# bartelvdh/Navtex

Measured on AMD Instinct MI355X. Metric: IQ Msamples/s through FIR->FSK->bitsync, higher is better.
Workload: dtype f64

## Files before the change

### navtex_amd/__init__.py

```python
from __future__ import annotations

import ctypes as C
import os
from typing import Callable, Iterable, List, Optional, Sequence, Tuple

import numpy as np

from . import _native as N
from ._native import (CHAIN_490, CHAIN_518, FRAME_BITS, FRAME_IN, FRAME_RAW, FRAME_Y3, RATE_IN, RATE_RAW,
                      SOFT_DECODE, SOFT_KEEP, NvxError, lib)

__all__ = ["Pipeline", "Group", "Capture", "Sitor", "sitor_encode", "make_stream", "synth_host", "synth_device", "device_count",
           "DeviceBuffer", "channelise", "channelise_time_stats", "Store", "wav_write", "wav_read", "NvxError", "lib",
           "CHAIN_518", "CHAIN_490", "SOFT_DECODE", "SOFT_KEEP", "FRAME_BITS", "FRAME_IN", "FRAME_RAW", "FRAME_Y3", "RATE_IN", "RATE_RAW"]


def device_count() -> int:
    return lib.nvx_device_count()


def sitor_encode(text: str, n_phasing: int = 40) -> str:
    t = text.encode("ascii")
    n = lib.nvx_sitor_encode(t, n_phasing, None, 0)
    buf = C.create_string_buffer(n + 1)
# ... 210 lines not shown
        N.check(lib.nvx_get_carrier(self._h, stream, chain, C.byref(off), C.byref(ref)), "nvx_get_carrier")
        return off.value, bool(ref.value)

    def afc_enable(self, stream: int, chain: int, cfg: Optional[N.AfcConfig] = None, **fields) -> None:
        _afc_enable(lib.nvx_afc_enable, self._h, stream, chain, cfg, fields, "nvx_afc_enable")

    def afc_disable(self, stream: int, chain: int, keep: bool = False) -> None:
        N.check(lib.nvx_afc_disable(self._h, stream, chain, int(keep)), "nvx_afc_disable")

    def afc_status(self, stream: int, chain: int) -> dict:
        return _afc_status(lib.nvx_afc_read, self._h, stream, chain, "nvx_afc_read")

    def afc_trace(self, stream: int, chain: int) -> List[int]:
        return _afc_trace(lib.nvx_afc_trace, self._h, stream, chain, "nvx_afc_trace")

    def set_forms(self, independent: int = -1, dynamic_preroll: int = -1, demod_tiles: int = -1) -> None:
        N.check(lib.nvx_debug_set_forms(self._h, independent, dynamic_preroll, demod_tiles), "nvx_debug_set_forms")

    def last_forms(self) -> Tuple[int, int, int]:
        a, b, c = C.c_int(), C.c_int(), C.c_int()
        N.check(lib.nvx_debug_last_forms(self._h, C.byref(a), C.byref(b), C.byref(c)), "nvx_debug_last_forms")
        return a.value, b.value, c.value

    def _apply_forms(self, forms: Optional[Sequence[int]]) -> None:
        if forms is None:
            if not hasattr(lib, "nvx_debug_set_forms"):
                return
            forms = tuple(int(os.environ.get(name, -1)) for name in ("NVX_INDEPENDENT", "NVX_DYNAMIC_PREROLL", "NVX_DEMOD_TILES"))
        if tuple(forms) != (-1, -1, -1):
            self.set_forms(*forms)


class Pipeline(HandleStats):

    def __init__(self, n_streams: int = 1, raw_rate: bool = False, chain_mask: int = CHAIN_518 | CHAIN_490,
                 chain_masks: Optional[Iterable[int]] = None, labels: Optional[Sequence[Sequence[int]]] = None,
                 max_frames: int = 1, char_layer: bool = True, push_mode: bool = False, device: int = 0,
                 wideband: bool = False, bit_history: int = 0, store: "Optional[Store]" = None, stage0_order: int = 1,
                 eager_launch: bool = False, stall_timeout_ms: int = 0, forms: Optional[Sequence[int]] = None):
        self.messages: List[Tuple[int, int, str, str]] = []
        cfg = N.Config()
        lib.nvx_config_default(C.byref(cfg))
        cfg.device, cfg.n_streams, cfg.raw_rate = device, n_streams, int(raw_rate)
        cfg.stage0_order = int(stage0_order)
        cfg.eager_launch = int(eager_launch)
        cfg.stall_timeout_ms = int(stall_timeout_ms)
        cfg.chain_mask, cfg.max_frames, cfg.char_layer, cfg.push_mode = chain_mask, max_frames, int(char_layer), int(push_mode)
# ... 362 lines not shown
```

### navtex_amd/_native.py

```python
from __future__ import annotations

import ctypes as C
import os
from pathlib import Path

import numpy as np

_LIB_PATH = Path(os.environ.get("NAVTEX_AMD_LIB") or (Path(__file__).resolve().parent / "libnavtex_amd.so"))

OK, ERR_ARG, ERR_NODEV, ERR_HIP, ERR_NOMEM, ERR_STATE, ERR_IO = 0, -1, -2, -3, -4, -5, -6
RATE_RAW, RATE_IN = 2016000, 252000
FRAME_BITS, FRAME_IN, FRAME_RAW, FRAME_Y3 = 32, 80640, 645120, 288
CHAIN_518, CHAIN_490 = 1, 2
SOFT_DECODE, SOFT_KEEP = 1, 2
TUNE_N, TUNE_STEP_HZ, TUNE_MAX_HZ, TUNE_NOMINAL_K = 20160, 3.125, 25000.0, 4480

MESSAGE_FN = C.CFUNCTYPE(None, C.c_void_p, C.c_int, C.c_char_p, C.c_char_p, C.c_int)
SITOR_MSG_FN = C.CFUNCTYPE(None, C.c_void_p, C.c_char_p, C.c_char_p, C.c_int)
SITOR_TRACE_FN = C.CFUNCTYPE(None, C.c_void_p, C.c_char_p)


class Config(C.Structure):
    _fields_ = [
        ("struct_size", C.c_uint32), ("device", C.c_int), ("n_streams", C.c_int), ("raw_rate", C.c_int), ("chain_mask", C.c_uint32),
# ... 30 lines not shown
                ("min_samples", C.c_int), ("contrast_min", C.c_double)]


class AfcStatus(C.Structure):
    _fields_ = [("enabled", C.c_int), ("centre_k", C.c_int), ("k_last", C.c_int), ("last_step", C.c_int), ("offset_hz", C.c_double),
                ("launches", C.c_uint64), ("updates", C.c_uint64), ("held", C.c_uint64), ("clamped", C.c_uint64)]


AFC_TRACE_KEEP = 1024


def _load() -> C.CDLL:
    if not _LIB_PATH.exists():
        raise ImportError(
            f"{_LIB_PATH} is missing: build it with `python navtex_amd/build.py` "
            "(hipcc, gfx950). navtex_amd has no pure-Python or CPU fallback.")
    lib = C.CDLL(str(_LIB_PATH))
    vp, sz, i, u32 = C.c_void_p, C.c_size_t, C.c_int, C.c_uint32
    sig = {
        "nvx_last_error": (C.c_char_p, []), "nvx_version": (C.c_char_p, []), "nvx_abi_version": (i, []),
        "nvx_sample_to_int16": (i, [C.c_double, C.POINTER(C.c_int16)]), "nvx_shim_stats": (i, [C.POINTER(C.c_uint64), C.POINTER(C.c_uint64)]),
        "nvx_debug_advance_clock": (i, [vp, i, C.c_uint64]),
        "nvx_debug_set_forms": (i, [vp, i, i, i]), "nvx_debug_last_forms": (i, [vp, C.POINTER(i), C.POINTER(i), C.POINTER(i)]),
        "init_fir_filter1": (None, []), "sample_in_1": (None, [C.c_double, C.c_double]), "init_fir2_wrapper": (None, []),
        "nvx_set_trace": (i, [vp, SITOR_TRACE_FN, vp]),
        "nvx_shim_latency": (i, [C.POINTER(C.c_uint64), C.POINTER(C.c_double), C.POINTER(C.c_double), C.POINTER(C.c_double), C.POINTER(C.c_double), i]),
        "nvx_shim_flush": (i, []), "nvx_shim_finish": (i, []), "nvx_shim_bits": (sz, [i, C.c_char_p, sz]),
        "nvx_StreamACallback": (None, [vp, vp, vp, C.c_uint, C.c_uint, vp]),
        "nvx_capture_start": (i, [vp, i, C.c_double, C.POINTER(vp)]), "nvx_capture_callback": (None, [vp, vp, vp, C.c_uint, C.c_uint, vp]),
        "nvx_capture_latency": (i, [vp, C.POINTER(C.c_uint64), C.POINTER(C.c_double), C.POINTER(C.c_double), C.POINTER(C.c_double), C.POINTER(C.c_double), i]),
        "nvx_capture_stop": (i, [vp]), "nvx_capture_record": (i, [vp, C.c_char_p]), "nvx_fsm_selftest": (i, [u32, i]),
        "nvx_cascade_wait_stats": (i, [vp, C.POINTER(C.c_uint64), C.POINTER(C.c_uint64), C.POINTER(C.c_uint64), i]),
        "nvx_debug_cascade_state": (i, [vp, i, vp, sz, i]),
        "nvx_cascade_integrity_stats": (i, [vp, C.POINTER(C.c_uint64), C.POINTER(C.c_uint64), C.POINTER(C.c_uint64), i]), "nvx_capture_pause": (None, [vp, i]),
        "nvx_capture_stats": (None, [vp, C.POINTER(C.c_uint64), C.POINTER(C.c_uint64), C.POINTER(C.c_uint64)]),
        "nvx_config_default": (None, [C.POINTER(Config)]),
        "nvx_create": (i, [C.POINTER(Config), C.POINTER(vp)]), "nvx_destroy": (None, [vp]), "nvx_reset": (i, [vp]), "nvx_stream_reset": (i, [vp, i]),
        "nvx_push_iq": (i, [vp, i, vp, sz]), "nvx_push_planar": (i, [vp, i, vp, vp, sz]), "nvx_flush": (i, [vp]),
        "nvx_finish": (i, [vp]), "nvx_stream_finish": (i, [vp, i]),
        "nvx_poll_bits": (sz, [vp, i, i, C.c_char_p, sz]),
        "nvx_process_resident": (i, [vp, vp, sz, sz, i, vp]), "nvx_fetch_bits": (i, [vp]),
        "nvx_bit_count": (sz, [vp, i, i]),
        "nvx_last_kernel_ms": (C.c_float, [vp, i]), "nvx_enable_timing": (None, [vp, i]), "nvx_enable_debug": (i, [vp, i]),
        "nvx_group_create": (i, [C.POINTER(C.c_int), i, C.POINTER(Config), C.POINTER(vp)]), "nvx_group_destroy": (None, [vp]),
        "nvx_group_reset": (i, [vp]), "nvx_group_size": (i, [vp]),
        "nvx_group_member": (i, [vp, i, C.POINTER(i), C.POINTER(i), C.POINTER(i), C.POINTER(vp)]), "nvx_group_member_of": (i, [vp, i]),
# ... 81 lines not shown
```

### navtex_amd/csrc/nvx_api.cpp

```cpp
#include "nvx_handle.h"
#include <chrono>
#include <cmath>
#include "navtex_amd_afc.h"
#include "navtex_amd_signal.h"
#include "navtex_amd_soft.h"
#include "navtex_amd_tune.h"
#include "nvx_fsm.h"

extern "C" hipError_t nvx_launch_afc_update(const nvx_afc_args *a, hipStream_t s) __attribute__((weak));
static_assert(NVX_AFC_LAW_C == NVX_AFC_C && NVX_AFC_K_MAX * NVX_TUNE_STEP_HZ == NVX_TUNE_MAX_HZ, "the law's constants are the header's");
static_assert(sizeof(nvx_afc_note) == 8 && sizeof(nvx_afc_par) == 32, "layouts of nvx_afc_law.h");

static thread_local char g_err[512] = "";
extern "C" void nvx_set_error(const char *fmt, ...)
{
    va_list ap; va_start(ap, fmt);
    vsnprintf(g_err, sizeof g_err, fmt, ap);
    va_end(ap);
}
extern "C" const char *nvx_last_error(void) { return g_err; }
int64_t nvx_now_ns()
{
    return std::chrono::duration_cast<std::chrono::nanoseconds>(std::chrono::steady_clock::now().time_since_epoch()).count();
}
#define NVX_STR2(x) #x
#define NVX_STR(x) NVX_STR2(x)
// ... 127 lines not shown
        (void)hipFree(r.d_soft); r.d_soft = nullptr;
        (void)hipHostFree(r.h_soft); r.h_soft = nullptr;
        r.soft = false;
    }
    for (auto &s : h->slots) {
        if (s.soft_sitor) { nvx_sitor_free(s.soft_sitor); s.soft_sitor = nullptr; }
        s.soft_outbox.clear();
        std::vector<float>().swap(s.soft);
        s.soft_base = s.soft_polled = 0; s.soft_count = 0;
    }
    for (auto it = h->sinks.begin(); it != h->sinks.end();)
        if ((*it)->soft) { delete *it; it = h->sinks.erase(it); } else ++it;
    h->soft_mode = 0; h->soft_cap = 0;
}

static void free_handle(nvx_handle *h)
{
    if (!h) return;
    const std::string err = g_err;
    (void)hipSetDevice(h->cfg.device);
    (void)drain(h);
    snprintf(g_err, sizeof g_err, "%s", err.c_str());
    free_debug(h);
    free_afc(h);
    free_signal(h);
    free_soft(h);
    for (auto it = h->made.rbegin(); it != h->made.rend(); ++it) {
        switch (it->first) {
        case HipRes::stream: (void)hipStreamDestroy((hipStream_t)it->second); break;
        case HipRes::event:  (void)hipEventDestroy((hipEvent_t)it->second); break;
        case HipRes::device: (void)hipFree(it->second); break;
        case HipRes::pinned: (void)hipHostFree(it->second); break;
        }
    }
    for (auto &s : h->slots)
        if (s.sitor) nvx_sitor_free(s.sitor);
    for (auto *c : h->sinks) delete c;
    delete h;
}

extern "C" void nvx_destroy(nvx_handle *h) { free_handle(h); }

extern "C" int nvx_create(const nvx_config *cfg, nvx_handle **out)
{
    if (!cfg || !out) { nvx_set_error("nvx_create: null argument"); return NVX_ERR_ARG; }
    *out = nullptr;
// ... 290 lines not shown
        ca.n_frames = n_frames; ca.n_streams = n_here; ca.chain_masks = h->d_masks;
        ca.part = d_list;
        ca.state[0] = h->d_cstate[p0]; ca.state[1] = h->d_cstate[p0 ^ 1]; ca.y3 = h->d_y3[yb]; ca.y3_cap = (size_t)h->y3_cap; ca.y3_base = 0;
        ca.queue = h->d_ctrl; ca.status = h->d_ctrl + 1; ca.done = h->d_ctrl + NVX_CASCADE_CTRL_INTS;
        ca.stage0_order = h->cfg.stage0_order;
        ca.third0 = third0;
        ca.tune_k = afc ? h->d_afc_k[h->launched & 1] : h->d_tune_k;
        ca.max_waves_per_cu = -1;
        HIP_TRY(nvx_launch_cascade(&ca, h->cascade_raw, h->nch, &forms, st));
    }
    if (r.timed) HIP_TRY(hipEventRecord(r.ev[1], st));
    HIP_TRY(hipMemcpyAsync(h->h_status + NVX_STATUS_INTS * (h->launched % RESULT_SLOTS), h->d_ctrl + 1, NVX_STATUS_INTS * sizeof(int), hipMemcpyDeviceToHost, st));
    HIP_TRY(hipEventRecord(h->casc_done[yb], st));
    HIP_TRY(hipStreamWaitEvent(sd, h->casc_done[yb], 0));
    if (fused) {
        nvx_fir3_args fa{};
        fa.y2[0] = y2_bufs[0]; fa.y2[1] = y2_bufs[1]; fa.y2_pitch = h->y2_pitch; fa.y2_row = h->d_y2row;
        fa.y3 = h->d_y3[yb]; fa.y3_cap = (size_t)h->y3_cap; fa.y3_base = 0; fa.n_frames = n_frames; fa.n_slots = h->n_slots;
        fa.part = d_list; fa.n_part = r.n_part; fa.per_part = h->per_in;
        if (r.timed) HIP_TRY(hipEventRecord(r.ev[6], sd));
        HIP_TRY(nvx_launch_fir3(&fa, sd));
        if (r.timed) HIP_TRY(hipEventRecord(r.ev[7], sd));
    }
    if (r.timed) HIP_TRY(hipEventRecord(r.ev[2], sd));
    HIP_TRY(nvx_launch_demod_front(&da, sd));
    if (r.timed) HIP_TRY(hipEventRecord(r.ev[3], sd));
    if (!da.soft && !afc) HIP_TRY(hipEventRecord(h->demod_done[yb], sd));
    h->demod_pending[yb] = true;
    if (r.timed) HIP_TRY(hipEventRecord(r.ev[4], sd));
    HIP_TRY(nvx_launch_demod_fsm(&da, sd));
    if (r.timed) HIP_TRY(hipEventRecord(r.ev[5], sd));
    if (afc) {
        nvx_afc_args aa{};
        aa.sig = r.d_sig; aa.par = h->d_afc_par; aa.k_rw = h->d_afc_k[h->launched & 1]; aa.k_next = h->d_afc_k[(h->launched + 1) & 1];
        aa.note = r.d_note; aa.n_slots = h->n_slots; aa.part = d_list; aa.n_part = r.n_part;
        if (r.timed) HIP_TRY(hipEventRecord(r.ev[8], sd));
        HIP_TRY(nvx_launch_afc_update(&aa, sd));
        if (r.timed) HIP_TRY(hipEventRecord(r.ev[9], sd));
    }
    if (da.soft || afc) HIP_TRY(hipEventRecord(h->demod_done[yb], sd));
    HIP_TRY(hipMemcpyAsync(h->h_ties, h->d_ties, sizeof(nvx_tie_stats), hipMemcpyDeviceToHost, sd));
    HIP_TRY(hipMemcpyAsync(r.h_nbits, r.d_nbits, (size_t)h->n_slots * sizeof(int), hipMemcpyDeviceToHost, sd));
    HIP_TRY(hipMemcpyAsync(r.h_bits, r.d_bits, (size_t)h->n_slots * h->bits_cap, hipMemcpyDeviceToHost, sd));
    if (h->sig_on) HIP_TRY(hipMemcpyAsync(r.h_sig, r.d_sig, (size_t)h->n_slots * sizeof(nvx_sig_rec), hipMemcpyDeviceToHost, sd));
    r.sig = h->sig_on;
    if (afc) HIP_TRY(hipMemcpyAsync(r.h_note, r.d_note, (size_t)h->n_slots * sizeof(nvx_afc_note), hipMemcpyDeviceToHost, sd));
// ... 674 lines not shown
    if (periods > (~0ull - g_old) / (unsigned long long)NVX_CLOCK_PERIOD) { nvx_set_error("nvx_debug_advance_clock: the clock would pass 2^64"); return NVX_ERR_ARG; }
    const unsigned long long g_new = g_old + periods * (unsigned long long)NVX_CLOCK_PERIOD;
    const unsigned third_old = (unsigned)(g_old / (NVX_FRAME_Y3 / 3)), third_new = (unsigned)(g_new / (NVX_FRAME_Y3 / 3));
    unsigned long long seal[2];
    uint8_t *entry = h->d_cstate[h->parity[stream]] + (size_t)stream * NVX_CASCADE_STATE_BYTES + (size_t)NVX_STATE_SEAL * 16;
    HIP_TRY(hipMemcpy(seal, entry, sizeof seal, hipMemcpyDeviceToHost));
    seal[0] ^= seal_tag_host(stream, third_old) ^ seal_tag_host(stream, third_new);
    seal[1] = ((unsigned long long)(unsigned)stream << 32) | third_new;
    HIP_TRY(hipMemcpy(entry, seal, sizeof seal, hipMemcpyHostToDevice));
    h->g0s[stream] = g_new;
    h->diverged = !streams_together(h);
    return NVX_OK;
}

extern "C" int nvx_debug_set_forms(nvx_handle *h, int independent, int dynamic_preroll, int demod_tiles)
{
    const auto bad = [](int v) { return v < -1 || v > 1; };
    if (!h || bad(independent) || bad(dynamic_preroll) || bad(demod_tiles)) { nvx_set_error("nvx_debug_set_forms: null handle, or a value outside -1 (automatic), 0, 1"); return NVX_ERR_ARG; }
    std::lock_guard<std::mutex> lk(h->mu);
    h->forms_req = nvx_forms{ independent, dynamic_preroll, demod_tiles };
    return NVX_OK;
}

extern "C" int nvx_debug_last_forms(nvx_handle *h, int *independent, int *dynamic_preroll, int *front_tile_wgs)
{
    if (!h) { nvx_set_error("nvx_debug_last_forms: null handle"); return NVX_ERR_ARG; }
    std::lock_guard<std::mutex> lk(h->mu);
    if (!h->forms_known) { nvx_set_error("nvx_debug_last_forms: the handle has launched nothing yet"); return NVX_ERR_STATE; }
    if (independent) *independent = h->forms_last.independent;
    if (dynamic_preroll) *dynamic_preroll = h->forms_last.dynamic_preroll;
    if (front_tile_wgs) *front_tile_wgs = h->forms_last.demod_tiles;
    return NVX_OK;
}

extern "C" size_t nvx_debug_y3(nvx_handle *h, int stream, int chain, double *out, size_t cap_pairs)
{
    if (!h || !out || stream < 0 || stream >= h->n_streams || chain < 0 || chain > 1) return 0;
    std::lock_guard<std::mutex> lk(h->mu);
    hipSetDevice(h->cfg.device);
    hipDeviceSynchronize();
    size_t n = std::min(cap_pairs, (size_t)h->last_n3);
    const int in = stream / h->per_in;
    if (h->ended[in]) n = std::min(n, (size_t)(h->g0s[in] % NVX_FRAME_Y3));
    if (hipMemcpy(out, h->d_y3[(h->launched + 1) & 1] + (size_t)(2 * stream + chain) * h->y3_cap, n * sizeof(double2), hipMemcpyDeviceToHost) != hipSuccess) return 0;
    return n;
}
// ... 67 lines not shown
```

### navtex_amd/csrc/nvx_cascade.hip

```cpp
#include <hip/hip_runtime.h>
#include <stdint.h>
#include <stdlib.h>
#include <mutex>

#include "nvx_cascade_wave.h"
#include "nvx_tune_table.h"

__device__ double2 nvx_tune_tab[NVX_TUNE_TAB_ENTRIES];

__device__ __forceinline__ int add_low_halves(unsigned a, unsigned b)
{
    int r;
    asm("v_add_u32_sdwa %0, sext(%1), sext(%2) dst_sel:DWORD dst_unused:UNUSED_PAD src0_sel:WORD_0 src1_sel:WORD_0"
        : "=v"(r) : "v"(a), "v"(b));
    return r;
}
__device__ __forceinline__ int add_high_halves(unsigned a, unsigned b)
{
    int r;
    asm("v_add_u32_sdwa %0, sext(%1), sext(%2) dst_sel:DWORD dst_unused:UNUSED_PAD src0_sel:WORD_1 src1_sel:WORD_1"
        : "=v"(r) : "v"(a), "v"(b));
    return r;
}
__device__ __forceinline__ double stage0_component(u32x4 v, bool odd)
{
    const int sI = add_low_halves(v.x, v.y) + add_low_halves(v.z, v.w);
    const int sQ = add_high_halves(v.x, v.y) + add_high_halves(v.z, v.w);
    int mine = (odd ? sQ : sI) + 4;
// ... 240 lines not shown
template <bool RAW, int NCH>
__global__ __launch_bounds__(64) void nvx_fir_cascade(nvx_cascade_args a)
{
    if (RAW) cascade_wave_main<RAW, NCH, 1, const nvx_cascade_args &>(a);
    else cascade_wave_main<RAW, NCH, 1, const nvx_cascade_args>(a);
}

__global__ __launch_bounds__(64) __attribute__((amdgpu_waves_per_eu(3, 3))) void nvx_fir_cascade_cic3_1(nvx_cascade_args a) { cascade_wave_main<true, 1, 3, const nvx_cascade_args &>(a); }
__global__ __launch_bounds__(64) void nvx_fir_cascade_cic3_2(nvx_cascade_args a) { cascade_wave_main<true, 2, 3, const nvx_cascade_args &>(a); }

template <bool RAW, int NCH, int S0>
__global__ __launch_bounds__(64) void nvx_fir_cascade_list(nvx_cascade_args a)
{
    if (RAW) cascade_wave_main<RAW, NCH, S0, const nvx_cascade_args &, true>(a);
    else cascade_wave_main<RAW, NCH, S0, const nvx_cascade_args, true>(a);
}

template <bool RAW, int NCH, int S0, bool LIST> struct CascadeKernel { static constexpr auto fn = nvx_fir_cascade_list<RAW, NCH, S0>; };
template <bool RAW, int NCH> struct CascadeKernel<RAW, NCH, 1, false> { static constexpr auto fn = nvx_fir_cascade<RAW, NCH>; };
template <> struct CascadeKernel<true, 1, 3, false> { static constexpr auto fn = nvx_fir_cascade_cic3_1; };
template <> struct CascadeKernel<true, 2, 3, false> { static constexpr auto fn = nvx_fir_cascade_cic3_2; };

#define NVX_MAX_DEVICES 64
template <bool RAW, int NCH, int S0 = 1, bool LIST = false>
static hipError_t launch_cascade_as(const nvx_cascade_args *a, nvx_forms *f, hipStream_t s)
{
    static std::mutex mu;
    static int cus_of[NVX_MAX_DEVICES], fit_of[NVX_MAX_DEVICES];
    int n_cus = 0, fit_per_cu = 0;
    {
        int dev = 0;
        hipError_t e = hipGetDevice(&dev);
        if (e != hipSuccess) return e;
        std::lock_guard<std::mutex> lk(mu);
        const bool cached = dev >= 0 && dev < NVX_MAX_DEVICES && cus_of[dev] > 0;
        if (!cached) {
            int cus = 0, per_cu = 0;
            e = hipDeviceGetAttribute(&cus, hipDeviceAttributeMultiprocessorCount, dev);
            if (e == hipSuccess) e = hipOccupancyMaxActiveBlocksPerMultiprocessor(&per_cu, CascadeKernel<RAW, NCH, S0, LIST>::fn, 64, 0);
            if (e != hipSuccess) return e;
            n_cus = cus; fit_per_cu = per_cu > 0 ? per_cu : 1;
            if (dev >= 0 && dev < NVX_MAX_DEVICES) { cus_of[dev] = n_cus; fit_of[dev] = fit_per_cu; }
        } else {
            n_cus = cus_of[dev]; fit_per_cu = fit_of[dev];
        }
    }
    int per_cu = fit_per_cu;
    if (a->max_waves_per_cu > 0 && a->max_waves_per_cu < per_cu) per_cu = a->max_waves_per_cu;
    if (a->max_waves_per_cu < 0 && per_cu + a->max_waves_per_cu >= 4) per_cu += a->max_waves_per_cu;
    const int resident = n_cus * per_cu;
    nvx_cascade_args args = *a;
    args.independent = f->independent >= 0 ? f->independent : (a->n_streams < resident && a->n_frames > 1);
    const long long whole_units = (long long)a->n_streams * a->n_frames;
    const int split_frames = whole_units > resident ? 1 : ((args.independent && 3 * whole_units <= resident) ? a->n_frames : 0);
    args.split_from = a->n_frames - split_frames;
    const long long units = (long long)a->n_streams * (args.split_from + 3LL * split_frames);
    const unsigned grid = (unsigned)(units < resident ? units : resident);
    args.dynamic_preroll = f->dynamic_preroll != 0;
    f->independent = args.independent; f->dynamic_preroll = args.dynamic_preroll;
    hipLaunchKernelGGL((CascadeKernel<RAW, NCH, S0, LIST>::fn), dim3(grid), dim3(64), 0, s, args);
    return hipGetLastError();
}

static hipError_t tune_table_ready()
{
    static std::mutex mu;
    static bool done[NVX_MAX_DEVICES];
    int dev = 0;
    hipError_t e = hipGetDevice(&dev);
    if (e != hipSuccess) return e;
    if (dev < 0 || dev >= NVX_MAX_DEVICES) return hipErrorInvalidDevice;
    std::lock_guard<std::mutex> lk(mu);
    if (done[dev]) return hipSuccess;
    double2 *tab = (double2 *)calloc(NVX_TUNE_TAB_ENTRIES, sizeof(double2));
    if (!tab) return hipErrorOutOfMemory;
    for (int j = 0; j < NVX_TUNE_TAB_N; j++) nvx_tune_entry(j, &tab[j].x, &tab[j].y);
    for (int o = 0; o < NVX_MIX_N; o++) {
        const int j = (NVX_TUNE_NOMINAL_K * o) % NVX_TUNE_TAB_N;
        tab[NVX_TUNE_TAB_N + j] = double2{ NVX_MIX_CR[o], NVX_MIX_CI[o] };
        tab[2 * NVX_TUNE_TAB_N + (NVX_TUNE_TAB_N - j) % NVX_TUNE_TAB_N] = double2{ NVX_MIX_CR[o], -NVX_MIX_CI[o] };
    }
    e = hipMemcpyToSymbol(HIP_SYMBOL(nvx_tune_tab), tab, NVX_TUNE_TAB_ENTRIES * sizeof(double2), 0, hipMemcpyHostToDevice);
    free(tab);
// ... 20 lines not shown
```

### navtex_amd/csrc/nvx_demod.hip

```cpp
#include <hip/hip_runtime.h>
#include <stdint.h>
#include <stdlib.h>

#include "nvx_tables.h"
#include "nvx_atan2.h"
#include "nvx_fsm.h"
#include "nvx_kernels.h"

enum { DS_Y3 = 0, DS_DPHI = 8, DS_S = 16, DS_C = 24, DS_COUNT = 24 + 567 };
enum { DI_SYNCED = 0, DI_SYNC_OFF, DI_NEXT_SYNC_OFF, DI_PHASE, DI_PREV_OFFSET, DI_COUNT };
static_assert(DI_COUNT == NVX_DEMOD_INTS && DS_COUNT == NVX_DEMOD_DOUBLES && DI_PREV_OFFSET == NVX_DI_PREV_OFFSET &&
              DI_PHASE == NVX_DI_PHASE, "state layout");

#ifndef NVX_FRONT_THREADS
#define NVX_FRONT_THREADS 128
#endif
#ifndef DTL
#define DTL NVX_FRONT_TILE
static_assert(DTL % 9 == 0, "a tile is a whole number of bit periods");
#endif
#define FRONT_SLIDE ((567 + NVX_FRONT_THREADS - 1) / NVX_FRONT_THREADS)
#define G_DAB 8
#define G_CB 574
#define G_CSA 582

__device__ __forceinline__ double2 y3_at(const double2 *y3, const double *hist, int t)
{
    if (t >= 0) return y3[t];
    double2 r; r.x = hist[2 * (4 + t)]; r.y = hist[2 * (4 + t) + 1];
    return r;
// ... 129 lines not shown
    c.slot = chain_index; c.g0 = a.g0; c.n3 = a.n3;
    int parity = 0;
    if (a.part) {
        const int per = 2 * a.per_part, e = chain_index / per;
        c.slot = a.part[e].stream * per + (chain_index - e * per);
        c.g0 = a.part[e].g0; parity = a.part[e].parity; c.n3 = a.part[e].n3;
    }
    c.st_rd = (parity ? a.dstate[1] : a.dstate[0]) + (size_t)c.slot * NVX_DEMOD_DOUBLES;
    c.st_wr = (parity ? a.dstate[0] : a.dstate[1]) + (size_t)c.slot * NVX_DEMOD_DOUBLES;
    return c;
}

__device__ __forceinline__ void front_publish_ties(const nvx_demod_args &a, const FrontTies &t, unsigned *s_near, unsigned *s_evals, unsigned *s_minm, int tid)
{
    if (t.evals) { atomicAdd(s_near, t.near); atomicAdd(s_evals, t.evals); atomicMin(s_minm, __float_as_uint(t.minm)); }
    __syncthreads();
    if (tid == 0 && *s_evals) {
        if (*s_near) atomicAdd(&a.ties->near_ties, (unsigned long long)*s_near);
        atomicAdd(&a.ties->evaluations, (unsigned long long)*s_evals);
        atomicMin(&a.ties->min_margin_bits, *s_minm);
    }
}

struct FrontWalkLds {
    double dphi[8 + DTL];
    double S[8 + DTL];
    double C[567 + DTL];
    unsigned char D[DTL];
    unsigned near, evals, minm;
    FrontSig sig[NVX_FRONT_THREADS / 64];
};
template <bool SIG>
__device__ __forceinline__ void front_sequential(const nvx_demod_args &a, int chain_index, int n_tiles_here, FrontWalkLds &lds)
{
    double *const s_dphi = lds.dphi, *const s_S = lds.S, *const s_C = lds.C;
    unsigned char *const s_D = lds.D;
    unsigned &s_near = lds.near, &s_evals = lds.evals, &s_minm = lds.minm;
    const int tid = threadIdx.x;
    const FrontChain ch = front_chain(a, chain_index);
    const int slot = ch.slot;
    if (!a.slot_active[slot]) return;
    if (tid == 0) { s_near = 0; s_evals = 0; s_minm = 0x7f800000u; }
    FrontTies ties = front_ties_init();
    constexpr bool sig_on = SIG;
    FrontSig sig;
    front_sig_init(sig);

    const double *st = ch.st_rd;
    const double2 *y3 = a.y3 + (size_t)slot * a.y3_cap + a.y3_base;
    double *dphi_out = a.dphi ? a.dphi + (size_t)slot * a.y3_cap + a.y3_base : nullptr;
    double *corr_out = a.corr ? a.corr + (size_t)slot * a.y3_cap + a.y3_base : nullptr;
    double *csum_out = a.csum ? a.csum + (size_t)slot * a.y3_cap + a.y3_base : nullptr;
    const double *hist = st + DS_Y3;
    if (tid < 8) { s_dphi[tid] = st[DS_DPHI + tid]; s_S[tid] = st[DS_S + tid]; }
    for (int i = tid; i < 567; i += NVX_FRONT_THREADS) s_C[i] = st[DS_C + i];
    __syncthreads();

    const int n3 = ch.n3;
    const int n_here = n_tiles_here > 0 ? min(n3, n_tiles_here * DTL) : n3;
    for (int ta = 0; ta < n_here; ta += DTL) {
        const int tl = min(DTL, n_here - ta);
        const int tl9 = (tl + 8) / 9;
        const unsigned long long gt = ch.g0 + (unsigned long long)ta;
        for (int L = tid; L < tl; L += NVX_FRONT_THREADS) {
            const int t = ta + L;
            const double2 w3 = y3_at(y3, hist, t - 1), w4 = y3[t];
            const double ds = front_dphi(w4, w3);
            s_dphi[8 + L] = ds;
            if (dphi_out) dphi_out[t] = ds;
            float hi, lo;
            const unsigned char d = front_decision(y3_at(y3, hist, t - 4), y3_at(y3, hist, t - 3), y3_at(y3, hist, t - 2), w3, w4, hi, lo);
            s_D[L] = d;
            if (sig_on && gt + L >= G_DAB) front_sig_add(sig, w4, ds, d, hi, lo);
        }
        if (tid < 9 * tl9 - tl) s_D[tl + tid] = 0;
        __syncthreads();
        for (int L = tid; L < tl; L += NVX_FRONT_THREADS)
            s_C[567 + L] = (gt + L >= G_DAB) ? front_corr(&s_dphi[L]) : 0.0;
        __syncthreads();
        const unsigned t_cb = (unsigned)((gt % 5103u + (5103u - G_CB % 5103u)) % 5103u);
        for (int L = tid; L < tl; L += NVX_FRONT_THREADS)
            s_S[8 + L] = (gt + L >= G_CB) ? front_class_sum(&s_C[567 + L], t_cb + (unsigned)L) : 0.0;
        __syncthreads();
        if (corr_out)
            for (int L = tid; L < tl; L += NVX_FRONT_THREADS) { corr_out[ta + L] = s_C[567 + L]; csum_out[ta + L] = s_S[8 + L]; }
        for (int M = tid; M < tl9; M += NVX_FRONT_THREADS) {
            const int L = 9 * M + (G_CSA % 9);
// ... 3 lines not shown
        double h_d = 0.0, h_s = 0.0, h_c[FRONT_SLIDE];
        if (tid < 8) { h_d = s_dphi[tl + tid]; h_s = s_S[tl + tid]; }
#pragma unroll
        for (int k = 0; k < FRONT_SLIDE; k++) { const int i = tid + NVX_FRONT_THREADS * k; h_c[k] = (i < 567) ? s_C[tl + i] : 0.0; }
        __syncthreads();
        if (tid < 8) { s_dphi[tid] = h_d; s_S[tid] = h_s; }
#pragma unroll
        for (int k = 0; k < FRONT_SLIDE; k++) { const int i = tid + NVX_FRONT_THREADS * k; if (i < 567) s_C[i] = h_c[k]; }
        __syncthreads();
    }

    front_publish_ties(a, ties, &s_near, &s_evals, &s_minm, tid);
    if (sig_on) {
        const unsigned skip = ch.g0 >= G_DAB ? 0u : (unsigned)min((unsigned long long)n_here, G_DAB - ch.g0);
        front_sig_publish(sig, (unsigned)n_here - skip, lds.sig, a.sig_part + (size_t)slot * a.sig_stride, tid);
    }
    if (n_tiles_here > 0) return;
    double *sw = ch.st_wr;
    if (tid < 4 && n3 >= 4) { const double2 l = y3[n3 - 4 + tid]; sw[DS_Y3 + 2 * tid] = l.x; sw[DS_Y3 + 2 * tid + 1] = l.y; }
    if (tid < 8) { sw[DS_DPHI + tid] = s_dphi[tid]; sw[DS_S + tid] = s_S[tid]; }
    for (int i = tid; i < 567; i += NVX_FRONT_THREADS) sw[DS_C + i] = s_C[i];
}

__global__ __launch_bounds__(NVX_FRONT_THREADS) __attribute__((amdgpu_waves_per_eu(5))) void nvx_demod_front(nvx_demod_args a)
{
    __shared__ FrontWalkLds lds;
    if (a.sig) front_sequential<true>(a, blockIdx.x, 0, lds);
    else front_sequential<false>(a, blockIdx.x, 0, lds);
}

#define FRONT_LOOKBACK 576
__global__ __launch_bounds__(NVX_FRONT_THREADS) void nvx_demod_front_head(nvx_demod_args a)
{
    __shared__ FrontWalkLds lds;
    if (a.sig) front_sequential<true>(a, blockIdx.x, 2, lds);
    else front_sequential<false>(a, blockIdx.x, 2, lds);
}
__global__ __launch_bounds__(NVX_FRONT_THREADS) void nvx_demod_front_tiles(nvx_demod_args a, int wgs_per_chain)
{
    const int chain_index = blockIdx.x / wgs_per_chain, wg = blockIdx.x - chain_index * wgs_per_chain;
    __shared__ double p_dphi[FRONT_LOOKBACK + DTL];
    __shared__ double p_C[FRONT_LOOKBACK - 8 + DTL];
    __shared__ double p_S[2 + DTL];
    __shared__ unsigned char p_D[DTL];
    __shared__ unsigned s_near, s_evals, s_minm;
    __shared__ FrontSig s_sig[NVX_FRONT_THREADS / 64];
    const int tid = threadIdx.x;
    const FrontChain ch = front_chain(a, chain_index);
    const int slot = ch.slot;
    if (!a.slot_active[slot]) return;
    if (tid == 0) { s_near = 0; s_evals = 0; s_minm = 0x7f800000u; }
// ... 208 lines not shown
    {
        const uint4 *src = (const uint4 *)a.fsm_table;
        uint4 *dst = (uint4 *)s_tab;
        for (int i = threadIdx.x; i < NVX_FSM_TABLE_ALLOC / 4; i += 64) dst[i] = src[i];
    }
    __syncthreads();
    if (a.soft) fsm_chain<true>(a, s_tab);
    else fsm_chain<false>(a, s_tab);
}

extern "C" int nvx_front_tile_wgs(const nvx_demod_args *a, int request)
{
    const unsigned chains = a->part ? (unsigned)(2 * a->per_part * a->n_part) : (unsigned)a->n_slots;
    const int tiles = (a->n3 + DTL - 1) / DTL;
    const long long chain_frames = (long long)chains * (a->n3 / NVX_Y3_PER_FRAME);
    const bool parallel = tiles >= 3 && (request >= 0 ? request != 0 : chain_frames <= 2560);
    return parallel ? tiles - 2 : 0;
}

extern "C" hipError_t nvx_launch_demod_front(const nvx_demod_args *a, hipStream_t s)
{
    const unsigned chains = a->part ? (unsigned)(2 * a->per_part * a->n_part) : (unsigned)a->n_slots;
    const int wgs = a->sig_parts - 1;
    if (wgs < 0) return hipErrorInvalidValue;
    if (a->sig && 1 + wgs > a->sig_stride) return hipErrorInvalidValue;
    if (wgs) {
        hipLaunchKernelGGL(nvx_demod_front_head, dim3(chains), dim3(NVX_FRONT_THREADS), 0, s, *a);
        hipLaunchKernelGGL(nvx_demod_front_tiles, dim3(chains * (unsigned)wgs), dim3(NVX_FRONT_THREADS), 0, s, *a, wgs);
    } else {
        hipLaunchKernelGGL(nvx_demod_front, dim3(chains), dim3(NVX_FRONT_THREADS), 0, s, *a);
    }
    return hipGetLastError();
}

extern "C" hipError_t nvx_launch_demod_fsm(const nvx_demod_args *a, hipStream_t s)
{
    const int chains = a->part ? 2 * a->per_part * a->n_part : a->n_slots;
    if (a->sig_parts < 1) return hipErrorInvalidValue;
    hipLaunchKernelGGL(nvx_demod_fsm, dim3((unsigned)((chains + 63) / 64)), dim3(64), 0, s, *a);
    return hipGetLastError();
}

extern "C" __attribute__((visibility("default"))) double nvx_atan2_host(double y, double x) { return nvx_atan2(y, x); }
```

### navtex_amd/csrc/nvx_handle.h

```cpp
#ifndef NVX_HANDLE_H
#define NVX_HANDLE_H

#include <hip/hip_runtime.h>

#include <algorithm>
#include <atomic>
#include <condition_variable>
#include <cstdarg>
#include <cstdio>
#include <cstdlib>
#include <cstring>
#include <mutex>
#include <string>
#include <thread>
#include <vector>

#include "navtex_amd.h"
#include "nvx_internal.h"
#include "nvx_kernels.h"
#include "nvx_afc_law.h"
#include "nvx_pool.h"

#define HIP_TRY(expr)                                                                      \
    do {                                                                                   \
// ... 137 lines not shown
    int *d_di = nullptr;
    uint32_t *d_fsm_tab = nullptr;
    unsigned short *d_words = nullptr;
    nvx_tie_stats *d_ties = nullptr;
    nvx_tie_stats *h_ties = nullptr;
    int *d_ctrl = nullptr;
    int *h_status = nullptr;
    uint64_t wait_polls = 0, wait_units = 0, wait_launches = 0;
    uint64_t stale_repaired = 0, integrity_failures = 0;
    std::vector<uint8_t> parity;
    std::vector<unsigned long long> g0s;
    bool diverged = false;
    uint64_t partial_launches = 0;
    std::vector<uint8_t> ended;
    bool poisoned = false;
    std::string poison_why;
    Result res[RESULT_SLOTS];
    std::vector<ArrivalClock *> arrival;
    int n_arrival = 0;
    uint64_t launched = 0, collected = 0;
    int last_n3 = 0;
    nvx_forms forms_req = { -1, -1, -1 }, forms_last = { -1, -1, -1 };
    bool forms_known = false;
    bool timing = false;
    float ms[5] = { 0.f, 0.f, 0.f, 0.f, 0.f };
    double ms_sum[5] = { 0.0, 0.0, 0.0, 0.0, 0.0 };
    uint64_t ms_count = 0;
    std::vector<uint8_t> masks;
    std::vector<Slot> slots;
    std::vector<struct SinkCtx *> sinks;
    HostPool pool;
    std::vector<std::pair<HipRes, void *>> made;
    std::mutex mu;
    uint32_t *h_stage[2] = { nullptr, nullptr };
    std::vector<uint8_t> cur;
    std::vector<uint64_t> set_launch[2];
    uint64_t copies_synced = 0;
    std::vector<uint8_t> active;
    size_t stage_cap = 0;
    std::vector<size_t> fill;
    uint32_t *d_in = nullptr;
    std::vector<uint8_t> writing;
    std::vector<uint8_t> pushing;
    std::vector<uint8_t> closing;
    std::vector<int64_t> last_push_ns;
    std::vector<int64_t> stall_ns;
// ... 39 lines not shown
```

### navtex_amd/csrc/nvx_kernels.h

```cpp
#ifndef NVX_KERNELS_H
#define NVX_KERNELS_H

#include <hip/hip_runtime.h>
#include <stdint.h>
#include "nvx_synth.h"

#define NVX_PASSES_PER_FRAME 315
#define NVX_Y3_PER_FRAME 288
#define NVX_THIRD_PASSES (NVX_PASSES_PER_FRAME / 3)
#define NVX_THIRD_Y3 (NVX_Y3_PER_FRAME / 3)
#define NVX_Y2_PER_FRAME 2880
#define NVX_THIRD_Y2 (NVX_Y2_PER_FRAME / 3)
#define NVX_Y2_PREFIX 80
#define NVX_PREROLL_PASSES 9
#define NVX_PREROLL_U 96
#define NVX_PREROLL_Y2 64
#define NVX_CASCADE_CTRL_INTS 8
#define NVX_STATUS_TIMEOUT 1
#define NVX_STATUS_INTEGRITY 2
#define NVX_STATUS_INTS 4
#define NVX_STATE_DATA_ENTRIES (36 + 2 * (46 + 70))
#define NVX_STATE_CIC3 NVX_STATE_DATA_ENTRIES
#define NVX_STATE_SEAL (NVX_STATE_DATA_ENTRIES + 1)
#ifndef NVX_CASCADE_STATE_ENTRIES
// ... 71 lines not shown
    size_t y3_cap, y3_base;
    int n3;
    int n_slots;
    const uint8_t *slot_active;
    unsigned long long g0;
    const nvx_part *part;
    int n_part;
    int per_part;
    double *dstate[2];
    int *state_i;
    const uint32_t *fsm_table;
    unsigned short *words;
    uint8_t *bits; int bits_cap; int *nbits;
    double *dphi;
    double *corr, *csum;
    nvx_tie_stats *ties;
    nvx_sig_rec *sig;
    nvx_sig_rec *sig_part;
    int sig_stride;
    int sig_parts;
    float *soft;
    int soft_cap;
    unsigned short *soft_pos;
} nvx_demod_args;

typedef struct nvx_afc_par nvx_afc_par;
typedef struct nvx_afc_note nvx_afc_note;
typedef struct {
    const nvx_sig_rec *sig;
    const nvx_afc_par *par;
    int *k_rw;
    const int *k_next;
    nvx_afc_note *note;
    int n_slots;
    const nvx_part *part;
    int n_part;
} nvx_afc_args;

typedef struct {
    const nvx_synth_desc *desc;
    const nvx_period *pool;
    uint32_t *out; size_t pitch; size_t n; uint32_t spb;
} nvx_synth_args;

typedef struct {
    const uint32_t *raw;
// ... 9 lines not shown

#define NVX_WB_SUBBANDS_K 8
#define NVX_WB_HALO 40
typedef struct {
    const uint32_t *raw;
    size_t pitch, first_sample;
    int n_wide, n_frames;
    const nvx_part *part;
    const uint8_t *chain_masks;
    uint8_t *state[2];
    uint32_t *hist[2];
    double2 *y3; size_t y3_cap, y3_base;
    int *queue, *status, *done;
    int independent;
    int thirds;
    unsigned third0;
    double2 *y2[2]; size_t y2_pitch; const int *y2_row;
} nvx_wideband_args;

typedef struct {
    int independent;
    int dynamic_preroll;
    int demod_tiles;
} nvx_forms;

#ifdef __cplusplus
extern "C" {
#endif
hipError_t nvx_launch_wideband_fused(const nvx_wideband_args *a, nvx_forms *f, hipStream_t s);
hipError_t nvx_launch_channelise(const nvx_channelise_args *a, hipStream_t s);
hipError_t nvx_launch_cascade(const nvx_cascade_args *a, int raw, int nch, nvx_forms *f, hipStream_t s);
hipError_t nvx_launch_fir3(const nvx_fir3_args *a, hipStream_t s);
int nvx_front_tile_wgs(const nvx_demod_args *a, int request);
hipError_t nvx_launch_demod_front(const nvx_demod_args *a, hipStream_t s);
hipError_t nvx_launch_demod_fsm(const nvx_demod_args *a, hipStream_t s);
hipError_t nvx_launch_synth(const nvx_synth_args *a, int n_streams, hipStream_t s);
double nvx_atan2_host(double y, double x);
hipError_t nvx_launch_afc_update(const nvx_afc_args *a, hipStream_t s);
int nvx_afc_step_host(int gain_shift, int max_step, int range_k, int min_samples, double contrast_min, int kc, int k0, int k1,
                      unsigned samples, unsigned b_samples, double sum_dphi_b, double sum_dphi_y, double sum_mf_hi, double sum_mf_lo,
                      unsigned *flags);
#ifdef __cplusplus
}
#endif
#endif
```

Baseline: 1.529 million.

## Halve demod walk tile LDS, pad cascade LDS, add persistent front grid

The sequential demod front walk now steps in half tiles, which shrinks its LDS footprint to fit a fixed budget so its workgroups can co-reside beside cascade waves. The cascade launch optionally adds dynamic LDS padding to reserve that space when waves per CU are reduced by one. An optional persistent grid for the front kernel pulls chains from an atomic queue. Halving the tile doubles loop iterations and barriers, and the new grid and queue path only runs when explicitly requested.

Measured after the change: 1.534 million, median of 2. Within noise of the previous version (+0.3%).

```diff
diff --git a/include/navtex_amd_grid.h b/include/navtex_amd_grid.h
--- /dev/null
+++ b/include/navtex_amd_grid.h
@@ -0,0 +1,16 @@
+#ifndef NAVTEX_AMD_GRID_H
+#define NAVTEX_AMD_GRID_H
+
+#include "navtex_amd.h"
+
+#ifdef __cplusplus
+extern "C" {
+#endif
+
+NVX_API int   nvx_debug_set_front_grid(nvx_handle *h, int workgroups);
+NVX_API int   nvx_debug_last_grids(nvx_handle *h, int *front_grid, int *cascade_pad, int *cascade_waves_per_cu);
+
+#ifdef __cplusplus
+}
+#endif
+#endif
diff --git a/navtex_amd/__init__.py b/navtex_amd/__init__.py
--- a/navtex_amd/__init__.py
+++ b/navtex_amd/__init__.py
@@ -256,7 +256,15 @@
         N.check(lib.nvx_debug_last_forms(self._h, C.byref(a), C.byref(b), C.byref(c)), "nvx_debug_last_forms")
         return a.value, b.value, c.value
 
-    def _apply_forms(self, forms: Optional[Sequence[int]]) -> None:
+    def set_front_grid(self, workgroups: int = -1) -> None:
+        N.check(lib.nvx_debug_set_front_grid(self._h, workgroups), "nvx_debug_set_front_grid")
+
+    def last_grids(self) -> Tuple[int, int, int]:
+        a, b, c = C.c_int(), C.c_int(), C.c_int()
+        N.check(lib.nvx_debug_last_grids(self._h, C.byref(a), C.byref(b), C.byref(c)), "nvx_debug_last_grids")
+        return a.value, b.value, c.value
+
+    def _apply_forms(self,forms: Optional[Sequence[int]]) -> None:
         if forms is None:
             if not hasattr(lib, "nvx_debug_set_forms"):
                 return
diff --git a/navtex_amd/_native.py b/navtex_amd/_native.py
--- a/navtex_amd/_native.py
+++ b/navtex_amd/_native.py
@@ -76,6 +76,7 @@
         "nvx_sample_to_int16": (i, [C.c_double, C.POINTER(C.c_int16)]), "nvx_shim_stats": (i, [C.POINTER(C.c_uint64), C.POINTER(C.c_uint64)]),
         "nvx_debug_advance_clock": (i, [vp, i, C.c_uint64]),
         "nvx_debug_set_forms": (i, [vp, i, i, i]), "nvx_debug_last_forms": (i, [vp, C.POINTER(i), C.POINTER(i), C.POINTER(i)]),
+        "nvx_debug_set_front_grid": (i, [vp, i]), "nvx_debug_last_grids": (i, [vp, C.POINTER(i), C.POINTER(i), C.POINTER(i)]),
         "init_fir_filter1": (None, []), "sample_in_1": (None, [C.c_double, C.c_double]), "init_fir2_wrapper": (None, []),
         "nvx_set_trace": (i, [vp, SITOR_TRACE_FN, vp]),
         "nvx_shim_latency": (i, [C.POINTER(C.c_uint64), C.POINTER(C.c_double), C.POINTER(C.c_double), C.POINTER(C.c_double), C.POINTER(C.c_double), i]),
diff --git a/navtex_amd/csrc/nvx_api.cpp b/navtex_amd/csrc/nvx_api.cpp
--- a/navtex_amd/csrc/nvx_api.cpp
+++ b/navtex_amd/csrc/nvx_api.cpp
@@ -2,6 +2,7 @@
 #include <chrono>
 #include <cmath>
 #include "navtex_amd_afc.h"
+#include "navtex_amd_grid.h"
 #include "navtex_amd_signal.h"
 #include "navtex_amd_soft.h"
 #include "navtex_amd_tune.h"
@@ -175,6 +176,7 @@
     (void)drain(h);
     snprintf(g_err, sizeof g_err, "%s", err.c_str());
     free_debug(h);
+    (void)hipFree(h->d_front_queue); h->d_front_queue = nullptr;
     free_afc(h);
     free_signal(h);
     free_soft(h);
@@ -511,6 +513,9 @@
         HIP_TRY(nvx_launch_fir3(&fa, sd));
         if (r.timed) HIP_TRY(hipEventRecord(r.ev[7], sd));
     }
+    da.front_queue = h->d_front_queue;
+    da.front_grid = forms.demod_tiles || h->front_grid_req < 0 ? 0 : h->front_grid_req;
+    forms.front_grid = da.front_grid;
     if (r.timed) HIP_TRY(hipEventRecord(r.ev[2], sd));
     HIP_TRY(nvx_launch_demod_front(&da, sd));
     if (r.timed) HIP_TRY(hipEventRecord(r.ev[3], sd));
@@ -1231,6 +1236,30 @@
     return NVX_OK;
 }
 
+extern "C" int nvx_debug_set_front_grid(nvx_handle *h, int workgroups)
+{
+    if (!h || workgroups < -1 || workgroups > 65536) { nvx_set_error("nvx_debug_set_front_grid: null handle, or a value outside -1 (automatic), 0 (per chain), 1..65536"); return NVX_ERR_ARG; }
+    std::lock_guard<std::mutex> lk(h->mu);
+    if (workgroups > 0 && !h->d_front_queue) {
+        HIP_TRY(hipSetDevice(h->cfg.device));
+        const hipError_t e = hipMalloc(&h->d_front_queue, sizeof(int));
+        if (e != hipSuccess) { h->d_front_queue = nullptr; nvx_set_error("nvx_debug_set_front_grid: hipMalloc failed: %s", hipGetErrorString(e)); return NVX_ERR_NOMEM; }
+    }
+    h->front_grid_req = workgroups;
+    return NVX_OK;
+}
+
+extern "C" int nvx_debug_last_grids(nvx_handle *h, int *front_grid, int *cascade_pad, int *cascade_waves_per_cu)
+{
+    if (!h) { nvx_set_error("nvx_debug_last_grids: null handle"); return NVX_ERR_ARG; }
+    std::lock_guard<std::mutex> lk(h->mu);
+    if (!h->forms_known) { nvx_set_error("nvx_debug_last_grids: the handle has launched nothing yet"); return NVX_ERR_STATE; }
+    if (front_grid) *front_grid = h->forms_last.front_grid;
+    if (cascade_pad) *cascade_pad = h->forms_last.cascade_pad;
+    if (cascade_waves_per_cu) *cascade_waves_per_cu = h->forms_last.cascade_waves;
+    return NVX_OK;
+}
+
 extern "C" int nvx_debug_last_forms(nvx_handle *h, int *independent, int *dynamic_preroll, int *front_tile_wgs)
 {
     if (!h) { nvx_set_error("nvx_debug_last_forms: null handle"); return NVX_ERR_ARG; }
diff --git a/navtex_amd/csrc/nvx_cascade.hip b/navtex_amd/csrc/nvx_cascade.hip
--- a/navtex_amd/csrc/nvx_cascade.hip
+++ b/navtex_amd/csrc/nvx_cascade.hip
@@ -4,6 +4,7 @@
 #include <mutex>
 
 #include "nvx_cascade_wave.h"
+#include "nvx_cascade_lds.h"
 #include "nvx_tune_table.h"
 
 __device__ double2 nvx_tune_tab[NVX_TUNE_TAB_ENTRIES];
@@ -290,12 +291,24 @@
 template <> struct CascadeKernel<true, 2, 3, false> { static constexpr auto fn = nvx_fir_cascade_cic3_2; };
 
 #define NVX_MAX_DEVICES 64
+template <typename K>
+static int lds_pad_of(K kernel, int dev, int fit)
+{
+    hipFuncAttributes fa{};
+    int lds_per_cu = 0, with_pad = 0;
+    if (hipFuncGetAttributes(&fa, (const void *)kernel) != hipSuccess ||
+        hipDeviceGetAttribute(&lds_per_cu, hipDeviceAttributeMaxSharedMemoryPerMultiprocessor, dev) != hipSuccess) { (void)hipGetLastError(); return 0; }
+    const int pad = nvx_cascade_lds_pad((int)fa.sharedSizeBytes, lds_per_cu, fit, NVX_FRONT_LDS_BUDGET, NVX_LDS_GRANULE);
+    if (pad <= 0) return 0;
+    if (hipOccupancyMaxActiveBlocksPerMultiprocessor(&with_pad, kernel, 64, (size_t)pad) != hipSuccess) { (void)hipGetLastError(); return 0; }
+    return with_pad == fit - 1 ? pad : 0;
+}
 template <bool RAW, int NCH, int S0 = 1, bool LIST = false>
 static hipError_t launch_cascade_as(const nvx_cascade_args *a, nvx_forms *f, hipStream_t s)
 {
     static std::mutex mu;
-    static int cus_of[NVX_MAX_DEVICES], fit_of[NVX_MAX_DEVICES];
-    int n_cus = 0, fit_per_cu = 0;
+    static int cus_of[NVX_MAX_DEVICES], fit_of[NVX_MAX_DEVICES], pad_of[NVX_MAX_DEVICES];
+    int n_cus = 0, fit_per_cu = 0, pad_bytes = 0;
     {
         int dev = 0;
         hipError_t e = hipGetDevice(&dev);
@@ -308,14 +321,16 @@
             if (e == hipSuccess) e = hipOccupancyMaxActiveBlocksPerMultiprocessor(&per_cu, CascadeKernel<RAW, NCH, S0, LIST>::fn, 64, 0);
             if (e != hipSuccess) return e;
             n_cus = cus; fit_per_cu = per_cu > 0 ? per_cu : 1;
-            if (dev >= 0 && dev < NVX_MAX_DEVICES) { cus_of[dev] = n_cus; fit_of[dev] = fit_per_cu; }
+            pad_bytes = lds_pad_of(CascadeKernel<RAW, NCH, S0, LIST>::fn, dev, fit_per_cu);
+            if (dev >= 0 && dev < NVX_MAX_DEVICES) { cus_of[dev] = n_cus; fit_of[dev] = fit_per_cu; pad_of[dev] = pad_bytes; }
         } else {
-            n_cus = cus_of[dev]; fit_per_cu = fit_of[dev];
+            n_cus = cus_of[dev]; fit_per_cu = fit_of[dev]; pad_bytes = pad_of[dev];
         }
     }
     int per_cu = fit_per_cu;
     if (a->max_waves_per_cu > 0 && a->max_waves_per_cu < per_cu) per_cu = a->max_waves_per_cu;
     if (a->max_waves_per_cu < 0 && per_cu + a->max_waves_per_cu >= 4) per_cu += a->max_waves_per_cu;
+    const unsigned pad = (a->max_waves_per_cu == -1 && per_cu == fit_per_cu - 1) ? (unsigned)pad_bytes : 0u;
     const int resident = n_cus * per_cu;
     nvx_cascade_args args = *a;
     args.independent = f->independent >= 0 ? f->independent : (a->n_streams < resident && a->n_frames > 1);
@@ -326,7 +341,8 @@
     const unsigned grid = (unsigned)(units < resident ? units : resident);
     args.dynamic_preroll = f->dynamic_preroll != 0;
     f->independent = args.independent; f->dynamic_preroll = args.dynamic_preroll;
-    hipLaunchKernelGGL((CascadeKernel<RAW, NCH, S0, LIST>::fn), dim3(grid), dim3(64), 0, s, args);
+    f->cascade_pad = (int)pad; f->cascade_waves = per_cu;
+    hipLaunchKernelGGL((CascadeKernel<RAW, NCH, S0, LIST>::fn), dim3(grid), dim3(64), pad, s, args);
     return hipGetLastError();
 }
 
diff --git a/navtex_amd/csrc/nvx_cascade_lds.h b/navtex_amd/csrc/nvx_cascade_lds.h
--- /dev/null
+++ b/navtex_amd/csrc/nvx_cascade_lds.h
@@ -0,0 +1,25 @@
+#ifndef NVX_CASCADE_LDS_H
+#define NVX_CASCADE_LDS_H
+
+#define NVX_FRONT_LDS_BUDGET 10240
+#define NVX_LDS_GRANULE 1280
+
+static inline long long nvx_lds_alloc(long long bytes, int granule)
+{
+    return (bytes + granule - 1) / granule * granule;
+}
+
+static inline int nvx_cascade_lds_pad(int static_bytes, int lds_per_cu, int fit, int front_bytes, int granule)
+{
+    if (static_bytes <= 0 || lds_per_cu <= 0 || front_bytes < 0 || granule <= 0) return -1;
+    const int n = fit - 1;
+    if (n < 1) return -1;
+    long long total = nvx_lds_alloc((long long)lds_per_cu / (n + 1) + 1, granule);
+    const long long own = nvx_lds_alloc(static_bytes, granule);
+    if (total < own) total = own;
+    if (lds_per_cu / total != n) return -1;
+    if (n * total + nvx_lds_alloc(front_bytes, granule) > lds_per_cu) return -1;
+    return (int)(total - static_bytes);
+}
+
+#endif
diff --git a/navtex_amd/csrc/nvx_demod.hip b/navtex_amd/csrc/nvx_demod.hip
--- a/navtex_amd/csrc/nvx_demod.hip
+++ b/navtex_amd/csrc/nvx_demod.hip
@@ -6,6 +6,7 @@
 #include "nvx_atan2.h"
 #include "nvx_fsm.h"
 #include "nvx_kernels.h"
+#include "nvx_cascade_lds.h"
 
 enum { DS_Y3 = 0, DS_DPHI = 8, DS_S = 16, DS_C = 24, DS_COUNT = 24 + 567 };
 enum { DI_SYNCED = 0, DI_SYNC_OFF, DI_NEXT_SYNC_OFF, DI_PHASE, DI_PREV_OFFSET, DI_COUNT };
@@ -181,14 +182,23 @@
     }
 }
 
+#define WTL (DTL / 2)
+static_assert(2 * WTL == DTL && WTL % 9 == 0, "the walk's step: half a tile, whole bit periods");
 struct FrontWalkLds {
-    double dphi[8 + DTL];
-    double S[8 + DTL];
-    double C[567 + DTL];
-    unsigned char D[DTL];
+    double dphi[8 + WTL];
+    double S[8 + WTL];
+    double C[567 + WTL];
+    unsigned char D[WTL];
     unsigned near, evals, minm;
+    int next;
     FrontSig sig[NVX_FRONT_THREADS / 64];
 };
+static_assert(sizeof(FrontWalkLds) <= NVX_FRONT_LDS_BUDGET, "a workgroup of the walk fits beside the next launch's cascade waves");
+__device__ __forceinline__ int front_walk_first(int ta, int tid)
+{
+    const int o = (ta % DTL) % NVX_FRONT_THREADS;
+    return (tid + NVX_FRONT_THREADS - o) % NVX_FRONT_THREADS;
+}
 template <bool SIG>
 __device__ __forceinline__ void front_sequential(const nvx_demod_args &a, int chain_index, int n_tiles_here, FrontWalkLds &lds)
 {
@@ -217,11 +227,11 @@
 
     const int n3 = ch.n3;
     const int n_here = n_tiles_here > 0 ? min(n3, n_tiles_here * DTL) : n3;
-    for (int ta = 0; ta < n_here; ta += DTL) {
-        const int tl = min(DTL, n_here - ta);
+    for (int ta = 0; ta < n_here; ta += WTL) {
+        const int tl = min(WTL, n_here - ta);
         const int tl9 = (tl + 8) / 9;
         const unsigned long long gt = ch.g0 + (unsigned long long)ta;
-        for (int L = tid; L < tl; L += NVX_FRONT_THREADS) {
+        for (int L = front_walk_first(ta, tid); L < tl; L += NVX_FRONT_THREADS) {
             const int t = ta + L;
             const double2 w3 = y3_at(y3, hist, t - 1), w4 = y3[t];
             const double ds = front_dphi(w4, w3);
@@ -271,11 +281,26 @@
     for (int i = tid; i < 567; i += NVX_FRONT_THREADS) sw[DS_C + i] = s_C[i];
 }
 
+template <bool SIG>
+__device__ __forceinline__ void front_walk(const nvx_demod_args &a, FrontWalkLds &lds)
+{
+    const int chains = a.part ? 2 * a.per_part * a.n_part : a.n_slots;
+    int chain = blockIdx.x;
+    while (chain < chains) {
+        front_sequential<SIG>(a, chain, 0, lds);
+        if ((int)gridDim.x >= chains) break;
+        __syncthreads();
+        if (threadIdx.x == 0) lds.next = (int)gridDim.x + atomicAdd(a.front_queue, 1);
+        __syncthreads();
+        chain = __builtin_amdgcn_readfirstlane(lds.next);
+    }
+}
+
 __global__ __launch_bounds__(NVX_FRONT_THREADS) __attribute__((amdgpu_waves_per_eu(5))) void nvx_demod_front(nvx_demod_args a)
 {
     __shared__ FrontWalkLds lds;
-    if (a.sig) front_sequential<true>(a, blockIdx.x, 0, lds);
-    else front_sequential<false>(a, blockIdx.x, 0, lds);
+    if (a.sig) front_walk<true>(a, lds);
+    else front_walk<false>(a, lds);
 }
 
 #define FRONT_LOOKBACK 576
@@ -530,11 +555,18 @@
 {
     const unsigned chains = a->part ? (unsigned)(2 * a->per_part * a->n_part) : (unsigned)a->n_slots;
     const int wgs = a->sig_parts - 1;
-    if (wgs < 0) return hipErrorInvalidValue;
+    if (wgs < 0 || a->front_grid < 0) return hipErrorInvalidValue;
     if (a->sig && 1 + wgs > a->sig_stride) return hipErrorInvalidValue;
     if (wgs) {
         hipLaunchKernelGGL(nvx_demod_front_head, dim3(chains), dim3(NVX_FRONT_THREADS), 0, s, *a);
         hipLaunchKernelGGL(nvx_demod_front_tiles, dim3(chains * (unsigned)wgs), dim3(NVX_FRONT_THREADS), 0, s, *a, wgs);
+    } else if (a->front_grid > 0) {
+        if ((unsigned)a->front_grid < chains) {
+            if (!a->front_queue) return hipErrorInvalidValue;
+            hipError_t e = hipMemsetAsync(a->front_queue, 0, sizeof(int), s);
+            if (e != hipSuccess) return e;
+        }
+        hipLaunchKernelGGL(nvx_demod_front, dim3((unsigned)a->front_grid), dim3(NVX_FRONT_THREADS), 0, s, *a);
     } else {
         hipLaunchKernelGGL(nvx_demod_front, dim3(chains), dim3(NVX_FRONT_THREADS), 0, s, *a);
     }
diff --git a/navtex_amd/csrc/nvx_handle.h b/navtex_amd/csrc/nvx_handle.h
--- a/navtex_amd/csrc/nvx_handle.h
+++ b/navtex_amd/csrc/nvx_handle.h
@@ -183,6 +183,8 @@
     int last_n3 = 0;
     nvx_forms forms_req = { -1, -1, -1 }, forms_last = { -1, -1, -1 };
     bool forms_known = false;
+    int front_grid_req = -1;
+    int *d_front_queue = nullptr;
     bool timing = false;
     float ms[5] = { 0.f, 0.f, 0.f, 0.f, 0.f };
     double ms_sum[5] = { 0.0, 0.0, 0.0, 0.0, 0.0 };
diff --git a/navtex_amd/csrc/nvx_kernels.h b/navtex_amd/csrc/nvx_kernels.h
--- a/navtex_amd/csrc/nvx_kernels.h
+++ b/navtex_amd/csrc/nvx_kernels.h
@@ -117,6 +117,8 @@
     float *soft;
     int soft_cap;
     unsigned short *soft_pos;
+    int front_grid;
+    int *front_queue;
 } nvx_demod_args;
 
 typedef struct nvx_afc_par nvx_afc_par;
@@ -172,6 +174,9 @@
     int independent;
     int dynamic_preroll;
     int demod_tiles;
+    int cascade_pad;
+    int cascade_waves;
+    int front_grid;
 } nvx_forms;
 
 #ifdef __cplusplus
```
